# YuePanEdward/MULLS

Hardware: NVIDIA H100
Metric: scan-pair registrations/sec (120k-pt 64-beam) (higher is better)
Workload: dtype f32 geometry / f64 accumulation

## Files before the change

### mulls_b200/csrc/device_types.cuh

```cuda
#pragma once
#include <cstdint>
#include <cuda_runtime.h>

#include "../../include/mulls_b200/abi.h"
#include "search_core.cuh"

namespace mulls {

constexpr int kNumClasses = MULLS_NUM_CLASSES;
constexpr int kNumSegs = 2 * kNumClasses;
constexpr int kIterBlock = 128;
constexpr int kIngestBlock = 256;
constexpr int kTerms = 28;
constexpr int kMaxLevels = 12;
constexpr int kCoordBits = 12;
constexpr int kDedupMinSrc = 500;
constexpr unsigned kClaimFree = 0x7f7f7f7fu;
constexpr int kIterFlags = 256;

enum PairStatus : int { kRunning = 0, kNeedPosterior = 1, kDone = 2 };

struct ChunkDesc {
    uint32_t pair;
    uint32_t seg;
// ... 34 lines not shown
    uint32_t src_index_base[kNumClasses];
    uint32_t src_global_n[kNumClasses];
    int sharded;
};

struct PairState {
    double T_total[16];
    double T_inc[16];
    double x[6];
    double cofactor[36];
    double info[36];
    double sigma2;
    double ibb[6];
    float thre;
    float confidence;
    float origin[3];
    float h0, inv_h0;
    int n_levels;
    int status, code, iter, iters_entered, final_buf;
    int source_feature_points_count;
    int n_src[kNumClasses];
    int n_src_g[kNumClasses];
    int n_src_g_next[kNumClasses];
    int n_tgt[kNumClasses];
    uint32_t n_corr[kNumClasses];
    uint32_t n_corr_last[kNumClasses];
    uint32_t seg_count[kNumSegs];
    uint32_t seg_start[kNumSegs];
    uint32_t hash_entries[kNumClasses];
    uint32_t hash_base[kNumClasses];
    uint32_t hash_mask[kNumClasses];
    int bb_src[6];
    int bb_tgt[6];
    uint64_t alg_bytes;
    int kl_keep[kNumSegs];
    uint32_t kl_rank[kNumSegs];
    uint64_t kl_prefix[kNumSegs];
    uint32_t kl_hist[kNumSegs][256];
};

struct LoopCtl {
    int it;
    int n_it_chunks;
    int n_pairs;
    int trace_on;
    int max_iter;
    unsigned solved;
    unsigned n_live[2];
    unsigned work[4];
};

struct DeviceArrays {
    const float4 *in_aos;
    float4 *stg_pos;
    float4 *stg_nrm;
    uint64_t *keys_a, *keys_b;
    uint32_t *vals_a, *vals_b;
    float4 *tgt_pos, *tgt_nrm;
    float4 *src_pos[2], *src_nrm[2];
    int *src_prevj[2];
    float4 *src_cert[2];
    int *nn_idx;
    float *nn_d2;
    uint8_t *flags;
    int *corr_j;
    float *corr_w;
    unsigned *claim;
    HashEntry *hash;
    uint32_t hash_pool_entries;
    uint32_t *hash_used;
    uint32_t *blk_kept;
    double *partials;
    double *post_partials;
    PairConst *pc;
    PairState *ps;
    ChunkDesc *in_chunks;
    ChunkDesc *it_chunks;
    mulls_icp_trace *trace;
    int *xch_i32;
    double *xch_f64;
    LoopCtl *ctl;
    uint32_t *live_chunks;
    uint32_t live_stride;
    int *running;
    volatile int *h_running;
    volatile int *h_running_iter;
};

}
```

### mulls_b200/csrc/kernels_ingest.cuh

```cuda
#pragma once
#include "device_math.cuh"
#include "device_types.cuh"

namespace mulls {

template <bool kUndistort>
__global__ void __launch_bounds__(kIngestBlock, kUndistort ? 4 : 6) k_ingest_transform(DeviceArrays A) {
    const ChunkDesc cd = A.in_chunks[blockIdx.x];
    const PairConst &pc = A.pc[cd.pair];
    const uint32_t seg = cd.seg;
    const uint32_t local = cd.first + threadIdx.x;
    const bool valid = local < pc.in_n[seg];
    const bool is_src = seg >= kNumClasses;
    const int cls = seg % kNumClasses;
    float x = 0, y = 0, z = 0;
    if (valid) {
        const size_t gi = (size_t)pc.in_off[seg] + local;
        float nx, ny, nz, intensity, curvature = 0.0f;
        const uint32_t fmt = pc.in_fmt[seg];
        if (fmt == 0u) {
            const float4 *in = pc.in_ptr[seg] + 3 * (size_t)local;
            const float4 a = in[0];
            const float4 b = in[1];
            const float4 c = in[2];
            x = a.x, y = a.y, z = a.z;
            nx = b.x, ny = b.y, nz = b.z;
            intensity = c.x, curvature = c.y;
        } else {
            const float4 *in = pc.in_ptr[seg];
            const float4 a = in[local];
            x = a.x, y = a.y, z = a.z, intensity = a.w;
            if (fmt == 1u) {
                const float *nr = reinterpret_cast<const float *>(in + pc.in_n[seg]) + 3 * (size_t)local;
                nx = nr[0], ny = nr[1], nz = nr[2];
            } else {
                const float4 b = in[(size_t)pc.in_n[seg] + local];
                nx = b.x, ny = b.y, nz = b.z, curvature = b.w;
            }
        }
        if (is_src) {
            const double *t = pc.init;
            int n_apply = 1;
            if (kUndistort && pc.undistort) {
                if (cls == MULLS_VERTEX) {
                    n_apply = 2;
                } else {
                    const float curv = curvature;
                    if (!(curv < 0.0f || (double)curv > 1.0)) {
                        const double s = (double)curv;
                        double scale0, scale1;
                        if (pc.ud_linear) {
                            scale0 = 1.0 - s;
                            scale1 = s;
                        } else {
                            scale0 = sin((1.0 - s) * pc.ud_theta) / pc.ud_sin_theta;
                            scale1 = sin(s * pc.ud_theta) / pc.ud_sin_theta;
                        }
                        if (pc.ud_neg) scale1 = -scale1;
                        const double qx = scale1 * pc.ud_q[0], qy = scale1 * pc.ud_q[1], qz = scale1 * pc.ud_q[2],
                                     qw = scale0 + scale1 * pc.ud_q[3];
                        const double vx = x, vy = y, vz = z;
                        double ux = qy * vz - qz * vy, uy = qz * vx - qx * vz, uz = qx * vy - qy * vx;
                        ux += ux, uy += uy, uz += uz;
                        const double rx = vx + qw * ux + (qy * uz - qz * uy);
                        const double ry = vy + qw * uy + (qz * ux - qx * uz);
                        const double rz = vz + qw * uz + (qx * uy - qy * ux);
                        x = (float)(rx + s * pc.ud_t[0]);
                        y = (float)(ry + s * pc.ud_t[1]);
                        z = (float)(rz + s * pc.ud_t[2]);
                    }
                }
            }
            for (int rep = 0; rep < n_apply; ++rep) {
                const double px = x, py = y, pz = z, qx = nx, qy = ny, qz = nz;
                x = (float)(t[0] * px + t[1] * py + t[2] * pz + t[3]);
                y = (float)(t[4] * px + t[5] * py + t[6] * pz + t[7]);
                z = (float)(t[8] * px + t[9] * py + t[10] * pz + t[11]);
                nx = (float)(t[0] * qx + t[1] * qy + t[2] * qz);
                ny = (float)(t[4] * qx + t[5] * qy + t[6] * qz);
                nz = (float)(t[8] * qx + t[9] * qy + t[10] * qz);
            }
        }
        A.stg_pos[gi] = make_float4(x, y, z, intensity);
        A.stg_nrm[gi] = make_float4(nx, ny, nz, __int_as_float((int)local));
    }
    const bool want = is_src ? (cls == MULLS_GROUND || cls == MULLS_PILLAR || cls == MULLS_FACADE) : true;
    if (!want) return;
    float mn[3] = {valid ? x : FLT_MAX, valid ? y : FLT_MAX, valid ? z : FLT_MAX};
    float mx[3] = {valid ? x : -FLT_MAX, valid ? y : -FLT_MAX, valid ? z : -FLT_MAX};
#pragma unroll
    for (int d = 0; d < 3; ++d)
#pragma unroll
        for (int o = 16; o > 0; o >>= 1) {
            mn[d] = fminf(mn[d], __shfl_xor_sync(0xffffffffu, mn[d], o));
            mx[d] = fmaxf(mx[d], __shfl_xor_sync(0xffffffffu, mx[d], o));
        }
    __shared__ float s_mn[kIngestBlock / 32][3], s_mx[kIngestBlock / 32][3];
    if ((threadIdx.x & 31) == 0) {
#pragma unroll
        for (int d = 0; d < 3; ++d) s_mn[threadIdx.x >> 5][d] = mn[d], s_mx[threadIdx.x >> 5][d] = mx[d];
    }
    __syncthreads();
    if (threadIdx.x < 6) {
        const int d = threadIdx.x % 3;
        const bool is_max = threadIdx.x >= 3;
        float v = is_max ? s_mx[0][d] : s_mn[0][d];
        for (int w = 1; w < kIngestBlock / 32; ++w) v = is_max ? fmaxf(v, s_mx[w][d]) : fminf(v, s_mn[w][d]);
        int *bb = is_src ? A.ps[cd.pair].bb_src : A.ps[cd.pair].bb_tgt;
        if (is_max) atomicMax(&bb[3 + d], float_to_ordered(v));
        else atomicMin(&bb[d], float_to_ordered(v));
    }
}

constexpr float kH0Min = 0.125f;
__global__ void k_pair_setup(DeviceArrays A, int n_pairs) {
    const int p = blockIdx.x * blockDim.x + threadIdx.x;
    if (p >= n_pairs) return;
    const PairConst &pc = A.pc[p];
    PairState &ps = A.ps[p];
    double smin[3], smax[3], tmin[3], tmax[3];
    for (int d = 0; d < 3; ++d) {
        smin[d] = (double)ordered_to_float(ps.bb_src[d]);
        smax[d] = (double)ordered_to_float(ps.bb_src[3 + d]);
        tmin[d] = (double)ordered_to_float(ps.bb_tgt[d]);
        tmax[d] = (double)ordered_to_float(ps.bb_tgt[3 + d]);
    }
    const double big = 1.7976931348623157e308;
    double gmin[3], gmax[3];
    if (pc.apply_filter) {
        const float pad = 1.0f;
        for (int d = 0; d < 3; ++d) {
            double lo = (pc.tbound[d] > smin[d]) ? pc.tbound[d] : smin[d];
            double hi = (pc.tbound[3 + d] < smax[d]) ? pc.tbound[3 + d] : smax[d];
            ps.ibb[d] = lo - (double)pad;
            ps.ibb[3 + d] = hi + (double)pad;
            gmin[d] = fmax(tmin[d], ps.ibb[d]);
            gmax[d] = fmin(tmax[d], ps.ibb[3 + d]);
        }
    } else {
        for (int d = 0; d < 3; ++d) {
            ps.ibb[d] = -big;
            ps.ibb[3 + d] = big;
            gmin[d] = tmin[d];
            gmax[d] = tmax[d];
        }
    }
    double ext = 0.0;
    for (int d = 0; d < 3; ++d) {
        if (!(gmax[d] >= gmin[d])) {
            gmin[d] = 0.0;
            gmax[d] = 0.0;
        }
        ext = fmax(ext, gmax[d] - gmin[d]);
    }
    const int ncell = 1 << kCoordBits;
    float h0 = kH0Min;
    while ((ext + 8.0 * h0) * 1.001 > (double)h0 * (ncell - 4)) h0 *= 2.0f;
    ps.h0 = h0;
    ps.inv_h0 = 1.0f / h0;
    for (int d = 0; d < 3; ++d) ps.origin[d] = (float)gmin[d] - 2.0f * h0;
    const float rmax = 2.5f * pc.thre_unit * 1.0001f;
    int L = 2;
    while (L < kMaxLevels && 0.999f * 0.5f * h0 * (float)(1 << (L - 1)) < rmax) ++L;
    if (pc.normal_shooting) L = kMaxLevels;
    ps.n_levels = L;

    for (int i = 0; i < 16; ++i) {
        ps.T_total[i] = pc.init[i];
        ps.T_inc[i] = (i % 5 == 0) ? 1.0 : 0.0;
    }
    for (int i = 0; i < 36; ++i) ps.cofactor[i] = ps.info[i] = (i % 7 == 0) ? 1.0 : 0.0;
    for (int i = 0; i < 6; ++i) ps.x[i] = 0.0;
    ps.sigma2 = 1.0;
    ps.thre = pc.thre_unit;
    ps.confidence = 1.0f;
    ps.status = kRunning;
    ps.code = 0;
    ps.iter = 0;
    ps.iters_entered = 0;
    ps.final_buf = 0;
    ps.alg_bytes = 0;
    if (pc.max_iter <= 0) {
        ps.status = kDone;
        const int left = atomicSub(A.running, 1) - 1;
        *A.h_running = left;
        __threadfence_system();
    }
}

__global__ void __launch_bounds__(kIngestBlock) k_make_keys(DeviceArrays A) {
    const ChunkDesc cd = A.in_chunks[blockIdx.x];
    const PairConst &pc = A.pc[cd.pair];
    PairState &ps = A.ps[cd.pair];
    const uint32_t seg = cd.seg;
    const uint32_t local = cd.first + threadIdx.x;
    const bool valid = local < pc.in_n[seg];
    bool inside = false;
    if (valid) {
        const size_t gi = (size_t)pc.in_off[seg] + local;
        const float4 p = A.stg_pos[gi];
        const double *b = ps.ibb;
        inside = (double)p.x > b[0] && (double)p.x < b[3] && (double)p.y > b[1] && (double)p.y < b[4] &&
                 (double)p.z > b[2] && (double)p.z < b[5];
        uint64_t key = ~0ull;
        if (inside) {
            const int hi = (1 << kCoordBits) - 1;
            int cx = (int)floorf((p.x - ps.origin[0]) * ps.inv_h0);
            int cy = (int)floorf((p.y - ps.origin[1]) * ps.inv_h0);
            int cz = (int)floorf((p.z - ps.origin[2]) * ps.inv_h0);
            cx = min(max(cx, 0), hi);
            cy = min(max(cy, 0), hi);
            cz = min(max(cz, 0), hi);
            key = ((uint64_t)(cd.pair * kNumSegs + seg) << 36) | morton36((uint32_t)cx, (uint32_t)cy, (uint32_t)cz);
        }
        A.keys_a[gi] = key;
        A.vals_a[gi] = (uint32_t)gi;
    }
    const unsigned ballot = __ballot_sync(0xffffffffu, inside);
    if ((threadIdx.x & 31) == 0 && ballot) atomicAdd(&ps.seg_count[seg], (unsigned)__popc(ballot));
}

__device__ __forceinline__ uint64_t sample_key(uint32_t seed, uint32_t cloud_id, uint32_t index) {
    uint64_t z = (((uint64_t)seed << 40) ^ ((uint64_t)cloud_id << 32) ^ (uint64_t)index) + 0x9e3779b97f4a7c15ull;
    z = (z ^ (z >> 30)) * 0xbf58476d1ce4e5b9ull;
    z = (z ^ (z >> 27)) * 0x94d049bb133111ebull;
    return z ^ (z >> 31);
}

__global__ void k_keepless_plan(DeviceArrays A, int n_pairs) {
    const int p = blockIdx.x * blockDim.x + threadIdx.x;
    if (p >= n_pairs) return;
    const PairConst &pc = A.pc[p];
    PairState &ps = A.ps[p];
    for (int s = 0; s < kNumSegs; ++s) {
        ps.kl_keep[s] = -1;
        ps.kl_prefix[s] = 0;
        ps.kl_rank[s] = 0;
        for (int b = 0; b < 256; ++b) ps.kl_hist[s][b] = 0;
    }
    if (!pc.keep_less) return;
    const int S = kNumClasses;
    auto plan = [&](int seg, int keep) {
        if ((int)ps.seg_count[seg] > keep) {
            ps.kl_keep[seg] = keep;
            ps.kl_rank[seg] = (uint32_t)keep;
        }
        return ((int)ps.seg_count[seg] > keep) ? keep : (int)ps.seg_count[seg];
    };
    const int tg = plan(MULLS_GROUND, (int)(ps.seg_count[MULLS_GROUND] / 2));
    const int tf = plan(MULLS_FACADE, (int)(ps.seg_count[MULLS_FACADE] / 2));
    plan(S + MULLS_GROUND, tg / 4);
    plan(S + MULLS_FACADE, tf / 2);
    plan(S + MULLS_PILLAR, (int)ps.seg_count[MULLS_PILLAR]);
// ... 65 lines not shown
}

__global__ void k_seg_offsets(DeviceArrays A, int n_pairs) {
    __shared__ uint32_t carry;
    __shared__ uint32_t warp_sums[32];
    if (threadIdx.x == 0) carry = 0;
    __syncthreads();
    const int total = n_pairs * kNumSegs;
    for (int base = 0; base < total; base += blockDim.x) {
        const int i = base + threadIdx.x;
        uint32_t v = 0;
        if (i < total) v = A.ps[i / kNumSegs].seg_count[i % kNumSegs];
        uint32_t incl = v;
        for (int o = 1; o < 32; o <<= 1) {
            uint32_t t = __shfl_up_sync(0xffffffffu, incl, o);
            if ((threadIdx.x & 31) >= o) incl += t;
        }
        if ((threadIdx.x & 31) == 31) warp_sums[threadIdx.x >> 5] = incl;
        __syncthreads();
        if (threadIdx.x < 32) {
            uint32_t w = (threadIdx.x < (blockDim.x >> 5)) ? warp_sums[threadIdx.x] : 0;
            uint32_t wi = w;
            for (int o = 1; o < 32; o <<= 1) {
                uint32_t t = __shfl_up_sync(0xffffffffu, wi, o);
                if (threadIdx.x >= o) wi += t;
            }
            warp_sums[threadIdx.x] = wi - w;
        }
        __syncthreads();
        const uint32_t excl = carry + warp_sums[threadIdx.x >> 5] + incl - v;
        if (i < total) A.ps[i / kNumSegs].seg_start[i % kNumSegs] = excl;
        __syncthreads();
        if (threadIdx.x == blockDim.x - 1) carry = excl + v;
        __syncthreads();
    }
    for (int p = threadIdx.x; p < n_pairs; p += blockDim.x) {
        PairState &ps = A.ps[p];
        const PairConst &pc = A.pc[p];
        for (int c = 0; c < kNumClasses; ++c) {
            ps.n_tgt[c] = (int)ps.seg_count[c];
            ps.n_src[c] = (int)ps.seg_count[kNumClasses + c];
            ps.n_src_g[c] = ps.n_src[c];
            ps.n_corr[c] = 0;
            ps.n_corr_last[c] = 0;
        }
        int cnt = 0;
        if (pc.used[MULLS_PILLAR]) cnt += ps.n_src[MULLS_PILLAR];
        if (pc.used[MULLS_FACADE]) cnt += ps.n_src[MULLS_FACADE];
        if (pc.used[MULLS_BEAM]) cnt += ps.n_src[MULLS_BEAM];
        ps.source_feature_points_count = cnt;
    }
}

__global__ void __launch_bounds__(256) k_gather(DeviceArrays A, const uint64_t *keys, const uint32_t *vals, uint32_t n_total) {
    const uint32_t i = blockIdx.x * blockDim.x + threadIdx.x;
    if (i >= n_total) return;
    const uint64_t key = keys[i];
    if (key == ~0ull) return;
    const uint32_t sg = (uint32_t)(key >> 36);
    const uint32_t pair = sg / kNumSegs, seg = sg % kNumSegs;
    const PairConst &pc = A.pc[pair];
    const uint32_t local = i - A.ps[pair].seg_start[seg];
    const uint32_t v = vals[i];
    const float4 pos = A.stg_pos[v];
    const float4 nrm = A.stg_nrm[v];
    if (seg < kNumClasses) {
        const uint32_t d = pc.tgt_base[seg] + local;
        A.tgt_pos[d] = pos;
        A.tgt_nrm[d] = nrm;
    } else {
        const uint32_t d = pc.src_base[seg - kNumClasses] + local;
        float4 n2 = nrm;
        if (pc.sharded) n2.w = __int_as_float(__float_as_int(nrm.w) + (int)pc.src_index_base[seg - kNumClasses]);
        A.src_pos[0][d] = pos;
        A.src_nrm[0][d] = n2;
        A.src_prevj[0][d] = -1;
        A.src_cert[0][d] = make_float4(0.f, 0.f, 0.f, 0.f);
    }
}

__device__ __forceinline__ void hash_insert(HashEntry *table, uint32_t mask, uint32_t klo, uint32_t khi, uint32_t start) {
    uint32_t slot = cell_hash(klo, khi) & mask;
    const unsigned long long packed = (unsigned long long)klo | ((unsigned long long)khi << 32);
    while (true) {
        unsigned long long *kp = reinterpret_cast<unsigned long long *>(&table[slot]);
        unsigned long long old = atomicCAS(kp, 0ull, packed);
        if (old == 0ull) {
            table[slot].start = start;
            return;
        }
        slot = (slot + 1) & mask;
    }
}
__device__ __forceinline__ HashEntry *hash_find(HashEntry *table, uint32_t mask, uint32_t klo, uint32_t khi) {
    uint32_t slot = cell_hash(klo, khi) & mask;
    while (true) {
        const uint32_t lo = *reinterpret_cast<volatile uint32_t *>(&table[slot].key_lo);
        const uint32_t hi = *reinterpret_cast<volatile uint32_t *>(&table[slot].key_hi);
        if (lo == klo && (hi & kKeyHiMask) == khi) return &table[slot];
        if (lo == 0u && hi == 0u) return nullptr;
        slot = (slot + 1) & mask;
    }
}

__global__ void __launch_bounds__(256) k_hash_build(DeviceArrays A, const uint64_t *keys, uint32_t n_total, int mode) {
    const uint32_t i = blockIdx.x * blockDim.x + threadIdx.x;
    const bool in_range = i <= n_total;
    const uint64_t kcur = (in_range && i < n_total) ? keys[i] : ~0ull;
    const uint64_t kprev = (in_range && i > 0) ? keys[i - 1] : ~0ull;
    const bool cur_t = kcur != ~0ull && ((uint32_t)(kcur >> 36) % kNumSegs) < kNumClasses;
    const bool prev_t = kprev != ~0ull && ((uint32_t)(kprev >> 36) % kNumSegs) < kNumClasses;
    const bool same_seg = cur_t && prev_t && (kcur >> 36) == (kprev >> 36);
    const uint64_t mmask = (1ull << 36) - 1;
    int top = kMaxLevels - 1;
    bool boundary = true;
    if (same_seg) {
        const uint64_t diff = (kcur ^ kprev) & mmask;
        if (diff == 0) boundary = false;
        else top = (63 - __clzll((long long)diff)) / 3;
    }
    if (mode == 0) {
        uint32_t sg = cur_t ? (uint32_t)(kcur >> 36) : 0xffffffffu;
        int cnt = 0;
        if (cur_t && boundary) {
            const int L = A.ps[sg / kNumSegs].n_levels;
            cnt = min(top, L - 1) + 1;
        }
        const unsigned grp = __match_any_sync(0xffffffffu, sg);
        if (grp == 0xffffffffu) {
            const int tot = __reduce_add_sync(0xffffffffu, cnt);
            if ((threadIdx.x & 31) == 0 && tot > 0 && cur_t)
                atomicAdd(&A.ps[sg / kNumSegs].hash_entries[sg % kNumSegs], (unsigned)tot);
        } else if (cnt > 0) {
            atomicAdd(&A.ps[sg / kNumSegs].hash_entries[sg % kNumSegs], (unsigned)cnt);
        }
        return;
    }
    if (!boundary || A.hash_used[1]) return;
    if (mode == 1) {
        if (!cur_t) return;
        const uint32_t sg = (uint32_t)(kcur >> 36);
        const uint32_t pair = sg / kNumSegs, cls = sg % kNumSegs;
        const PairState &ps = A.ps[pair];
        const int L = ps.n_levels;
        const uint32_t local = i - ps.seg_start[cls];
        HashEntry *table = A.hash + ps.hash_base[cls];
        const uint64_t m = kcur & mmask;
        const uint32_t x0 = compact12(m), y0 = compact12(m >> 1), z0 = compact12(m >> 2);
        for (int l = 0; l <= top && l < L; ++l)
            hash_insert(table, ps.hash_mask[cls], cell_key_lo(x0 >> l, y0 >> l, z0 >> l), cell_key_hi(z0 >> l, l), local);
    } else {
        if (!prev_t) return;
        const uint32_t sg = (uint32_t)(kprev >> 36);
        const uint32_t pair = sg / kNumSegs, cls = sg % kNumSegs;
        const PairState &ps = A.ps[pair];
        const int L = ps.n_levels;
        const uint32_t local_end = i - ps.seg_start[cls];
        HashEntry *table = A.hash + ps.hash_base[cls];
        const uint64_t m = kprev & mmask;
        const uint32_t x0 = compact12(m), y0 = compact12(m >> 1), z0 = compact12(m >> 2);
        for (int l = 0; l <= top && l < L; ++l) {
            const uint32_t x = x0 >> l, y = y0 >> l, z = z0 >> l;
            HashEntry *e = hash_find(table, ps.hash_mask[cls], cell_key_lo(x, y, z), cell_key_hi(z, l));
            if (e) e->count = local_end - e->start;
            if (l + 1 < L) {
                HashEntry *par = hash_find(table, ps.hash_mask[cls], cell_key_lo(x >> 1, y >> 1, z >> 1), cell_key_hi(z >> 1, l + 1));
                if (par) atomicOr(&par->key_hi, 1u << (16 + ((x & 1u) | ((y & 1u) << 1) | ((z & 1u) << 2))));
            }
        }
    }
}

constexpr uint64_t kHashSlack = 4;
__global__ void k_hash_layout(DeviceArrays A, int n_pairs) {
    if (threadIdx.x != 0 || blockIdx.x != 0) return;
    for (int attempt = 0; attempt < 3; ++attempt) {
        uint64_t used = 0;
        bool overflow = false;
        for (int p = 0; p < n_pairs && !overflow; ++p) {
            PairState &ps = A.ps[p];
            for (int c = 0; c < kNumClasses; ++c) {
                const uint64_t want = (attempt == 0) ? kHashSlack * ps.hash_entries[c] : (attempt == 1) ? 2ull * ps.hash_entries[c] : (5ull * ps.hash_entries[c]) / 4 + 1;
                uint32_t cap = 16;
                while (cap < want) cap <<= 1;
                if (used + cap > A.hash_pool_entries) {
                    overflow = true;
                    break;
                }
                ps.hash_base[c] = (uint32_t)used;
                ps.hash_mask[c] = cap - 1;
                used += cap;
            }
        }
        A.hash_used[0] = overflow ? 0u : (uint32_t)used;
        A.hash_used[1] = overflow ? 1u : 0u;
        if (!overflow) return;
    }
    for (int p = 0; p < n_pairs; ++p)
        for (int c = 0; c < kNumClasses; ++c) {
            A.ps[p].hash_base[c] = 0;
            A.ps[p].hash_mask[c] = 0;
        }
}

__global__ void __launch_bounds__(256) k_hash_clear(DeviceArrays A) {
    const uint32_t used = A.hash_used[0];
    const uint4 z = make_uint4(0, 0, 0, 0);
    for (uint32_t i = blockIdx.x * blockDim.x + threadIdx.x; i < used; i += gridDim.x * blockDim.x)
        reinterpret_cast<uint4 *>(A.hash)[i] = z;
}

}
```

### mulls_b200/csrc/mulls_b200.cu

```cuda
#include <algorithm>
#include <atomic>
#include <memory>
#include <cmath>
#include <cstdio>
#include <chrono>
#include <cstring>
#include <string>
#include <vector>

#include <cub/device/device_radix_sort.cuh>
#include <cub/device/device_scan.cuh>

#include <dlfcn.h>
#include <mutex>

#include "device_types.cuh"
#include "host_pack.h"
#include "scan_io.h"
#include "kernels_ingest.cuh"
#include "kernels_iterate.cuh"
#include "kernels_pca.cuh"
#include "kernels_map.cuh"
#include "kernels_classify.cuh"
#include "kernels_ground.cuh"
// ... 189 lines not shown
    if (ctx->graph) cudaGraphDestroy(ctx->graph);
    if (ctx->h_stage) cudaFreeHost(ctx->h_stage);
    for (cudaEvent_t e : ctx->ev_done) cudaEventDestroy(e);
    for (cudaEvent_t e : ctx->ev_search) cudaEventDestroy(e);
    if (ctx->ev_begin) cudaEventDestroy(ctx->ev_begin);
    if (ctx->ev_ingest) cudaEventDestroy(ctx->ev_ingest);
    if (ctx->ev_iter) cudaEventDestroy(ctx->ev_iter);
    if (ctx->ev_end) cudaEventDestroy(ctx->ev_end);
    if (ctx->ev_h2d0) cudaEventDestroy(ctx->ev_h2d0);
    if (ctx->stream) cudaStreamDestroy(ctx->stream);
    delete ctx;
}

mulls_ctx *mulls_create(int device, size_t max_pairs, size_t max_src_pts, size_t max_tgt_pts) {
    int ndev = 0;
    cudaError_t e = cudaGetDeviceCount(&ndev);
    if (e != cudaSuccess || ndev == 0) {
        g_create_error = std::string("mulls_create: no CUDA device (") + cudaGetErrorString(e) +
                         "); mulls_b200 has no CPU fallback";
        return nullptr;
    }
    if (device < 0 || device >= ndev || max_pairs == 0) {
        g_create_error = "mulls_create: bad device index or max_pairs";
        return nullptr;
    }
    mulls_ctx *ctx = new mulls_ctx();
    ctx->device = device;
    ctx->max_pairs = max_pairs;
    ctx->max_src = max_src_pts;
    ctx->max_tgt = max_tgt_pts;
    auto fail = [&](const char *what, cudaError_t err) -> mulls_ctx * {
        g_create_error = std::string("mulls_create: ") + what + ": " + cudaGetErrorString(err);
        mulls_destroy(ctx);
        return nullptr;
    };
    if ((e = cudaSetDevice(device)) != cudaSuccess) return fail("cudaSetDevice", e);
    if ((e = cudaStreamCreateWithFlags(&ctx->stream, cudaStreamNonBlocking)) != cudaSuccess) return fail("stream", e);
    const size_t cs = ctx->cap_src = max_pairs * max_src_pts;
    const size_t ct = ctx->cap_tgt = max_pairs * max_tgt_pts;
    const size_t cin = ctx->cap_in = cs + ct;
    if (cin >= (1ull << 31)) {
        g_create_error = "mulls_create: more than 2^31 points per context";
        mulls_destroy(ctx);
        return nullptr;
    }
    ctx->cap_it_chunks = ceil_div(cs, kIterBlock) + max_pairs * (kNumClasses + 1);
    ctx->cap_in_chunks = ceil_div(cin, kIngestBlock) + max_pairs * kNumSegs;
    DeviceArrays &A = ctx->A;
    float4 *in = nullptr;
#define ALLOC(ptr, n)                                                   \
    if ((e = dev_alloc(ctx, &(ptr), (n))) != cudaSuccess) return fail(#ptr, e)
    ALLOC(in, 3 * cin);
    A.in_aos = in;
    ALLOC(A.stg_pos, cin);
    ALLOC(A.stg_nrm, cin);
    ALLOC(A.keys_a, cin);
    ALLOC(A.keys_b, cin);
    ALLOC(A.vals_a, cin);
    ALLOC(A.vals_b, cin);
    ALLOC(A.tgt_pos, ct + kScanOverrun);
    ALLOC(A.tgt_nrm, ct);
    for (int b = 0; b < 2; ++b) {
        ALLOC(A.src_pos[b], cs);
        ALLOC(A.src_nrm[b], cs);
        ALLOC(A.src_prevj[b], cs);
        ALLOC(A.src_cert[b], cs);
    }
    ALLOC(A.nn_idx, cs);
    ALLOC(A.nn_d2, cs);
    ALLOC(A.flags, cs);
    ALLOC(A.corr_j, cs);
    ALLOC(A.corr_w, cs);
    ALLOC(A.claim, ct);
    {
        size_t pool = 12 * ct + 64 * max_pairs * kNumClasses;
        if (pool >= (1ull << 32)) pool = (1ull << 32) - 1;
        A.hash_pool_entries = (uint32_t)pool;
        ALLOC(A.hash, pool);
    }
    ALLOC(A.hash_used, 2);
    ALLOC(A.ctl, 1);
    ALLOC(A.blk_kept, ctx->cap_it_chunks);
    ALLOC(A.partials, ctx->cap_it_chunks * kTerms);
    ALLOC(A.post_partials, ctx->cap_it_chunks * 2);
    ALLOC(A.pc, max_pairs);
    ALLOC(A.ps, max_pairs);
    ALLOC(A.in_chunks, ctx->cap_in_chunks);
    ALLOC(A.it_chunks, ctx->cap_it_chunks);
    ALLOC(A.live_chunks, 2 * ctx->cap_it_chunks);
    A.live_stride = (uint32_t)ctx->cap_it_chunks;
    {
        int sms = 0;
        if (cudaDeviceGetAttribute(&sms, cudaDevAttrMultiProcessorCount, device) != cudaSuccess || sms <= 0) sms = 132;
        ctx->num_sms = sms;
    }
    ALLOC(ctx->d_results, max_pairs + ceil_div(max_pairs * sizeof(uint64_t), sizeof(mulls_icp_result)) + 1);
    ALLOC(ctx->d_trace, max_pairs);
    ALLOC(A.running, 1);
    ALLOC(A.xch_i32, 32);
    ALLOC(A.xch_f64, kNumClasses * kTerms + 8);
#undef ALLOC
    if ((e = cudaHostAlloc((void **)&ctx->h_running, (1 + kIterFlags) * sizeof(int), cudaHostAllocMapped)) != cudaSuccess)
        return fail("mapped flag", e);
    {
        int *dptr = nullptr;
        if ((e = cudaHostGetDevicePointer((void **)&dptr, ctx->h_running, 0)) != cudaSuccess) return fail("mapped flag", e);
        A.h_running = dptr;
        A.h_running_iter = dptr + 1;
// ... 312 lines not shown
        CK(ce);
    } else {
    if (cudaEventRecord(ctx->ev_h2d0, ctx->stream) == cudaSuccess) ctx->h2d_timed = true;
    for (size_t p = 0; p < n_pairs; ++p) {
        PairConst &pc = ctx->h_pc[p];
        for (int s = 0; s < kNumSegs; ++s) {
            const mulls_cloud_view &v = (s < kNumClasses) ? tgt[p * kNumClasses + s] : src[p * kNumClasses + (s - kNumClasses)];
            pc.in_ptr[s] = ctx->A.in_aos + 3 * (size_t)pc.in_off[s];
            pc.in_fmt[s] = kFmtRows48;
            if (v.n == 0) continue;
            if (tgt_on_device && s < kNumClasses) {
                pc.in_ptr[s] = (const float4 *)v.aos48;
                continue;
            }
            CK(cudaMemcpyAsync((void *)(ctx->A.in_aos + 3 * (size_t)pc.in_off[s]), v.aos48, v.n * 48, cudaMemcpyHostToDevice,
                               ctx->stream));
        }
    }
    }
    if (!tables_sent) {
        CK(cudaMemcpyAsync(ctx->A.pc, ctx->h_pc.data(), n_pairs * sizeof(PairConst), cudaMemcpyHostToDevice, ctx->stream));
        if (!ctx->h_in_chunks.empty())
            CK(cudaMemcpyAsync(ctx->A.in_chunks, ctx->h_in_chunks.data(), ctx->h_in_chunks.size() * sizeof(ChunkDesc),
                               cudaMemcpyHostToDevice, ctx->stream));
        if (!ctx->h_it_chunks.empty())
            CK(cudaMemcpyAsync(ctx->A.it_chunks, ctx->h_it_chunks.data(), ctx->h_it_chunks.size() * sizeof(ChunkDesc),
                               cudaMemcpyHostToDevice, ctx->stream));
    }
    if (resident) CK(cudaStreamSynchronize(ctx->stream));
    ctx->n_pairs = n_pairs;
    ctx->n_in = in_off;
    ctx->n_src_total = s_off;
    ctx->n_tgt_total = t_off;
    ctx->max_iter_max = max_iter_max;
    ctx->any_keep_less = any_keep_less;
    ctx->any_normal_shooting = any_shoot;
    ctx->any_undistort = any_undistort;
    ctx->uploaded = true;
    ctx->up_ms_host = (float)(wall_ms() - t_up0);
    return MULLS_OK;
}

static int launch_ingest(mulls_ctx *ctx, DeviceArrays &A, bool trace, uint64_t &launches, mulls_allreduce_fn hook = nullptr,
                         void *user = nullptr) {
    cudaStream_t st = ctx->stream;
    const int np = (int)ctx->n_pairs;
    const uint32_t n_in = (uint32_t)ctx->n_in;
    if (trace) CK(cudaMemsetAsync(ctx->d_trace, 0, np * sizeof(mulls_icp_trace), st));
    CK(cudaMemsetAsync(A.claim, 0x7f, std::max<size_t>(ctx->n_tgt_total, 1) * sizeof(unsigned), st));
    k_state_init<<<(unsigned)ceil_div(np, 128), 128, 0, st>>>(A, np);
    ++launches;
    const unsigned n_inc = (unsigned)ctx->h_in_chunks.size();
    if (n_inc) {
        if (ctx->any_undistort) k_ingest_transform<true><<<n_inc, kIngestBlock, 0, st>>>(A);
        else k_ingest_transform<false><<<n_inc, kIngestBlock, 0, st>>>(A);
        ++launches;
    }
    if (hook) {
        k_shard_pack_setup<<<1, 1, 0, st>>>(A, 0);
        if (hook(user, A.xch_i32, 6, 1, 1, (void *)st) != 0) {
            ctx->err = "all-reduce callback failed";
            return MULLS_E_COMM;
        }
        k_shard_pack_setup<<<1, 1, 0, st>>>(A, 1);
        launches += 2;
    }
    k_pair_setup<<<(unsigned)ceil_div(np, 128), 128, 0, st>>>(A, np);
    ++launches;
    if (n_inc) {
        k_make_keys<<<n_inc, kIngestBlock, 0, st>>>(A);
        ++launches;
        if (ctx->any_keep_less) {
            const unsigned pb = (unsigned)ceil_div(np, 64);
            k_keepless_plan<<<pb, 64, 0, st>>>(A, np);
            for (int pass = 0; pass < 8; ++pass) {
                k_keepless_hist<<<n_inc, kIngestBlock, 0, st>>>(A, pass);
                k_keepless_step<<<pb, 64, 0, st>>>(A, np, pass);
            }
            k_keepless_mark<<<n_inc, kIngestBlock, 0, st>>>(A);
            launches += 18;
        }
        int seg_bits = 1;
        while ((1ull << seg_bits) <= (uint64_t)np * kNumSegs) ++seg_bits;
        size_t bytes = ctx->cub_temp_bytes;
        CK(cub::DeviceRadixSort::SortPairs(ctx->cub_temp, bytes, A.keys_a, A.keys_b, A.vals_a, A.vals_b, (int)n_in, 0,
                                           36 + seg_bits, st));
    }
    k_seg_offsets<<<1, 256, 0, st>>>(A, np);
    ++launches;
    if (hook) {
        k_shard_pack_setup<<<1, 1, 0, st>>>(A, 2);
        if (hook(user, A.xch_i32, kNumClasses, 1, 0, (void *)st) != 0) {
            ctx->err = "all-reduce callback failed";
            return MULLS_E_COMM;
        }
        k_shard_pack_setup<<<1, 1, 0, st>>>(A, 3);
        launches += 2;
    }
    if (n_in) {
        k_gather<<<(unsigned)ceil_div(n_in, 256), 256, 0, st>>>(A, A.keys_b, A.vals_b, n_in);
        const unsigned hb = (unsigned)ceil_div((size_t)n_in + 1, 256);
        k_hash_build<<<hb, 256, 0, st>>>(A, A.keys_b, n_in, 0);
        k_hash_layout<<<1, 32, 0, st>>>(A, np);
        k_hash_clear<<<1184, 256, 0, st>>>(A);
        k_hash_build<<<hb, 256, 0, st>>>(A, A.keys_b, n_in, 1);
        k_hash_build<<<hb, 256, 0, st>>>(A, A.keys_b, n_in, 2);
        launches += 6;
    } else {
        k_hash_layout<<<1, 32, 0, st>>>(A, np);
        ++launches;
    }
    return MULLS_OK;
}

static unsigned chunk_bucket(const mulls_ctx *ctx) {
    unsigned b = 1;
    while (b < (unsigned)ctx->h_it_chunks.size()) b <<= 1;
    return b;
}
static unsigned resident_grid(const mulls_ctx *ctx, int blocks_per_sm) {
    return std::min((unsigned)(ctx->num_sms * blocks_per_sm), chunk_bucket(ctx));
}
static void launch_search(mulls_ctx *ctx, cudaStream_t st, const DeviceArrays &A, int buf, int it) {
    const unsigned grid = resident_grid(ctx, kSearchBlocksPerSm);
    const int mode = it < 0 ? -1 : (it >= kKeepFromIter ? 2 : (it == kKeepFromIter - 1 ? 1 : 0));
    if (mode < 0 || mode == 0) k_search<0><<<grid, kIterBlock, 0, st>>>(A, buf, it);
    if (mode < 0 || mode == 1) k_search<1><<<grid, kIterBlock, 0, st>>>(A, buf, it);
    if (mode < 0 || mode == 2) k_search<2><<<grid, kIterBlock, 0, st>>>(A, buf, it);
}
constexpr int kShootBlocksPerSm = 8, kResolveBlocksPerSm = 16, kAccumulateBlocksPerSm = 8;
constexpr int kPollPause = 64;

static int build_iteration_graph(mulls_ctx *ctx) {
    const int key[2] = {(int)chunk_bucket(ctx), ctx->any_normal_shooting ? 1 : 0};
    if (ctx->graph_exec && std::memcmp(key, ctx->graph_key, sizeof(key)) == 0) return MULLS_OK;
    if (ctx->graph_exec) cudaGraphExecDestroy(ctx->graph_exec), ctx->graph_exec = nullptr;
    if (ctx->graph) cudaGraphDestroy(ctx->graph), ctx->graph = nullptr;
    cudaStream_t st = ctx->stream;
    DeviceArrays A = ctx->A;
    const unsigned cap_chunks = (unsigned)std::max<size_t>(ctx->cap_it_chunks, 1), cap_pairs = (unsigned)std::max<size_t>(ctx->max_pairs, 1);
    CK(cudaGraphCreate(&ctx->graph, 0));
    cudaGraphConditionalHandle handle;
    CK(cudaGraphConditionalHandleCreate(&handle, ctx->graph, 1, cudaGraphCondAssignDefault));
    cudaGraphNodeParams wp = {cudaGraphNodeTypeConditional};
    wp.conditional.handle = handle;
    wp.conditional.type = cudaGraphCondTypeWhile;
    wp.conditional.size = 1;
    cudaGraphNode_t while_node;
    CK(cudaGraphAddNode(&while_node, ctx->graph, nullptr, 0, &wp));
    cudaGraph_t body = wp.conditional.phGraph_out[0];
    CK(cudaStreamBeginCaptureToGraph(st, body, nullptr, nullptr, 0, cudaStreamCaptureModeThreadLocal));
    launch_search(ctx, st, A, -1, -1);
    if (ctx->any_normal_shooting)
        k_search_shoot<<<resident_grid(ctx, kShootBlocksPerSm), kIterBlock, 0, st>>>(A, -1);
    k_resolve<<<resident_grid(ctx, kResolveBlocksPerSm), kIterBlock, 0, st>>>(A, -1);
    k_accumulate<<<resident_grid(ctx, kAccumulateBlocksPerSm), kIterBlock, 0, st>>>(A, -1);
    k_solve<<<cap_pairs, kSolveThreads, 0, st>>>(A, -1, (unsigned long long)handle);
    CK(cudaStreamEndCapture(st, nullptr));
    CK(cudaStreamBeginCaptureToGraph(st, ctx->graph, &while_node, nullptr, 1, cudaStreamCaptureModeThreadLocal));
    k_posterior<<<std::min(cap_chunks, chunk_bucket(ctx)), kIterBlock, 0, st>>>(A);
// ... 1301 lines not shown
```

Baseline: 5954.

## Drop staging buffers, recompute transforms on demand, and build hash in one pass

After: 6250 (median of 6 runs). +5.0%, better.

```diff
diff --git a/mulls_b200/csrc/device_types.cuh b/mulls_b200/csrc/device_types.cuh
--- a/mulls_b200/csrc/device_types.cuh
+++ b/mulls_b200/csrc/device_types.cuh
@@ -110,8 +110,6 @@
 
 struct DeviceArrays {
     const float4 *in_aos;
-    float4 *stg_pos;
-    float4 *stg_nrm;
     uint64_t *keys_a, *keys_b;
     uint32_t *vals_a, *vals_b;
     float4 *tgt_pos, *tgt_nrm;
diff --git a/mulls_b200/csrc/kernels_ingest.cuh b/mulls_b200/csrc/kernels_ingest.cuh
--- a/mulls_b200/csrc/kernels_ingest.cuh
+++ b/mulls_b200/csrc/kernels_ingest.cuh
@@ -4,90 +4,107 @@
 
 namespace mulls {
 
-template <bool kUndistort>
-__global__ void __launch_bounds__(kIngestBlock, kUndistort ? 4 : 6) k_ingest_transform(DeviceArrays A) {
-    const ChunkDesc cd = A.in_chunks[blockIdx.x];
-    const PairConst &pc = A.pc[cd.pair];
-    const uint32_t seg = cd.seg;
-    const uint32_t local = cd.first + threadIdx.x;
-    const bool valid = local < pc.in_n[seg];
+template <bool kUndistort, bool kNormals>
+__device__ __forceinline__ void load_input_point(const PairConst &pc, uint32_t seg, uint32_t local, float4 &pos, float4 &nrm) {
     const bool is_src = seg >= kNumClasses;
     const int cls = seg % kNumClasses;
-    float x = 0, y = 0, z = 0;
-    if (valid) {
-        const size_t gi = (size_t)pc.in_off[seg] + local;
-        float nx, ny, nz, intensity, curvature = 0.0f;
-        const uint32_t fmt = pc.in_fmt[seg];
-        if (fmt == 0u) {
-            const float4 *in = pc.in_ptr[seg] + 3 * (size_t)local;
-            const float4 a = in[0];
+    const bool undistort = kUndistort && is_src && pc.undistort && cls != MULLS_VERTEX;
+    float x, y, z, intensity = 0.0f, curvature = 0.0f;
+    float nx = 0.0f, ny = 0.0f, nz = 0.0f;
+    const uint32_t fmt = pc.in_fmt[seg];
+    if (fmt == 0u) {
+        const float4 *in = pc.in_ptr[seg] + 3 * (size_t)local;
+        const float4 a = in[0];
+        x = a.x, y = a.y, z = a.z;
+        if (kNormals) {
             const float4 b = in[1];
             const float4 c = in[2];
-            x = a.x, y = a.y, z = a.z;
             nx = b.x, ny = b.y, nz = b.z;
             intensity = c.x, curvature = c.y;
-        } else {
-            const float4 *in = pc.in_ptr[seg];
-            const float4 a = in[local];
-            x = a.x, y = a.y, z = a.z, intensity = a.w;
-            if (fmt == 1u) {
+        } else if (undistort) {
+            curvature = reinterpret_cast<const float *>(in + 2)[1];
+        }
+    } else {
+        const float4 *in = pc.in_ptr[seg];
+        const float4 a = in[local];
+        x = a.x, y = a.y, z = a.z, intensity = a.w;
+        if (fmt == 1u) {
+            if (kNormals) {
                 const float *nr = reinterpret_cast<const float *>(in + pc.in_n[seg]) + 3 * (size_t)local;
                 nx = nr[0], ny = nr[1], nz = nr[2];
+            }
+        } else if (kNormals) {
+            const float4 b = in[(size_t)pc.in_n[seg] + local];
+            nx = b.x, ny = b.y, nz = b.z, curvature = b.w;
+        } else if (undistort) {
+            curvature = in[(size_t)pc.in_n[seg] + local].w;
+        }
+    }
+    if (is_src) {
+        const double *t = pc.init;
+        int n_apply = 1;
+        if (kUndistort && pc.undistort) {
+            if (cls == MULLS_VERTEX) {
+                n_apply = 2;
             } else {
-                const float4 b = in[(size_t)pc.in_n[seg] + local];
-                nx = b.x, ny = b.y, nz = b.z, curvature = b.w;
-            }
-        }
-        if (is_src) {
-            const double *t = pc.init;
-            int n_apply = 1;
-            if (kUndistort && pc.undistort) {
-                if (cls == MULLS_VERTEX) {
-                    n_apply = 2;
-                } else {
-                    const float curv = curvature;
-                    if (!(curv < 0.0f || (double)curv > 1.0)) {
-                        const double s = (double)curv;
-                        double scale0, scale1;
-                        if (pc.ud_linear) {
-                            scale0 = 1.0 - s;
-                            scale1 = s;
-                        } else {
-                            scale0 = sin((1.0 - s) * pc.ud_theta) / pc.ud_sin_theta;
-                            scale1 = sin(s * pc.ud_theta) / pc.ud_sin_theta;
-                        }
-                        if (pc.ud_neg) scale1 = -scale1;
-                        const double qx = scale1 * pc.ud_q[0], qy = scale1 * pc.ud_q[1], qz = scale1 * pc.ud_q[2],
-                                     qw = scale0 + scale1 * pc.ud_q[3];
-                        const double vx = x, vy = y, vz = z;
-                        double ux = qy * vz - qz * vy, uy = qz * vx - qx * vz, uz = qx * vy - qy * vx;
-                        ux += ux, uy += uy, uz += uz;
-                        const double rx = vx + qw * ux + (qy * uz - qz * uy);
-                        const double ry = vy + qw * uy + (qz * ux - qx * uz);
-                        const double rz = vz + qw * uz + (qx * uy - qy * ux);
-                        x = (float)(rx + s * pc.ud_t[0]);
-                        y = (float)(ry + s * pc.ud_t[1]);
-                        z = (float)(rz + s * pc.ud_t[2]);
+                const float curv = curvature;
+                if (!(curv < 0.0f || (double)curv > 1.0)) {
+                    const double s = (double)curv;
+                    double scale0, scale1;
+                    if (pc.ud_linear) {
+                        scale0 = 1.0 - s;
+                        scale1 = s;
+                    } else {
+                        scale0 = sin((1.0 - s) * pc.ud_theta) / pc.ud_sin_theta;
+                        scale1 = sin(s * pc.ud_theta) / pc.ud_sin_theta;
                     }
+                    if (pc.ud_neg) scale1 = -scale1;
+                    const double qx = scale1 * pc.ud_q[0], qy = scale1 * pc.ud_q[1], qz = scale1 * pc.ud_q[2],
+                                 qw = scale0 + scale1 * pc.ud_q[3];
+                    const double vx = x, vy = y, vz = z;
+                    double ux = qy * vz - qz * vy, uy = qz * vx - qx * vz, uz = qx * vy - qy * vx;
+                    ux += ux, uy += uy, uz += uz;
+                    const double rx = vx + qw * ux + (qy * uz - qz * uy);
+                    const double ry = vy + qw * uy + (qz * ux - qx * uz);
+                    const double rz = vz + qw * uz + (qx * uy - qy * ux);
+                    x = (float)(rx + s * pc.ud_t[0]);
+                    y = (float)(ry + s * pc.ud_t[1]);
+                    z = (float)(rz + s * pc.ud_t[2]);
                 }
             }
-            for (int rep = 0; rep < n_apply; ++rep) {
-                const double px = x, py = y, pz = z, qx = nx, qy = ny, qz = nz;
-                x = (float)(t[0] * px + t[1] * py + t[2] * pz + t[3]);
-                y = (float)(t[4] * px + t[5] * py + t[6] * pz + t[7]);
-                z = (float)(t[8] * px + t[9] * py + t[10] * pz + t[11]);
+        }
+        for (int rep = 0; rep < n_apply; ++rep) {
+            const double px = x, py = y, pz = z;
+            x = (float)(t[0] * px + t[1] * py + t[2] * pz + t[3]);
+            y = (float)(t[4] * px + t[5] * py + t[6] * pz + t[7]);
+            z = (float)(t[8] * px + t[9] * py + t[10] * pz + t[11]);
+            if (kNormals) {
+                const double qx = nx, qy = ny, qz = nz;
                 nx = (float)(t[0] * qx + t[1] * qy + t[2] * qz);
                 ny = (float)(t[4] * qx + t[5] * qy + t[6] * qz);
                 nz = (float)(t[8] * qx + t[9] * qy + t[10] * qz);
             }
         }
-        A.stg_pos[gi] = make_float4(x, y, z, intensity);
-        A.stg_nrm[gi] = make_float4(nx, ny, nz, __int_as_float((int)local));
-    }
+    }
+    pos = make_float4(x, y, z, intensity);
+    if (kNormals) nrm = make_float4(nx, ny, nz, __int_as_float((int)local));
+}
+
+template <bool kUndistort>
+__global__ void __launch_bounds__(kIngestBlock) k_ingest_bbox(DeviceArrays A) {
+    const ChunkDesc cd = A.in_chunks[blockIdx.x];
+    const PairConst &pc = A.pc[cd.pair];
+    const uint32_t seg = cd.seg;
+    const bool is_src = seg >= kNumClasses;
+    const int cls = seg % kNumClasses;
     const bool want = is_src ? (cls == MULLS_GROUND || cls == MULLS_PILLAR || cls == MULLS_FACADE) : true;
     if (!want) return;
-    float mn[3] = {valid ? x : FLT_MAX, valid ? y : FLT_MAX, valid ? z : FLT_MAX};
-    float mx[3] = {valid ? x : -FLT_MAX, valid ? y : -FLT_MAX, valid ? z : -FLT_MAX};
+    const uint32_t local = cd.first + threadIdx.x;
+    const bool valid = local < pc.in_n[seg];
+    float4 p = make_float4(0.f, 0.f, 0.f, 0.f), unused;
+    if (valid) load_input_point<kUndistort, false>(pc, seg, local, p, unused);
+    float mn[3] = {valid ? p.x : FLT_MAX, valid ? p.y : FLT_MAX, valid ? p.z : FLT_MAX};
+    float mx[3] = {valid ? p.x : -FLT_MAX, valid ? p.y : -FLT_MAX, valid ? p.z : -FLT_MAX};
 #pragma unroll
     for (int d = 0; d < 3; ++d)
 #pragma unroll
@@ -188,6 +205,7 @@
     }
 }
 
+template <bool kUndistort>
 __global__ void __launch_bounds__(kIngestBlock) k_make_keys(DeviceArrays A) {
     const ChunkDesc cd = A.in_chunks[blockIdx.x];
     const PairConst &pc = A.pc[cd.pair];
@@ -198,7 +216,8 @@
     bool inside = false;
     if (valid) {
         const size_t gi = (size_t)pc.in_off[seg] + local;
-        const float4 p = A.stg_pos[gi];
+        float4 p, unused;
+        load_input_point<kUndistort, false>(pc, seg, local, p, unused);
         const double *b = ps.ibb;
         inside = (double)p.x > b[0] && (double)p.x < b[3] && (double)p.y > b[1] && (double)p.y < b[4] &&
                  (double)p.z > b[2] && (double)p.z < b[5];
@@ -370,122 +389,114 @@
     }
 }
 
+__device__ __forceinline__ int cell_top(const uint64_t *keys, uint32_t i, uint64_t kcur) {
+    if (kcur == ~0ull || ((uint32_t)(kcur >> 36) % kNumSegs) >= kNumClasses) return -1;
+    if (i == 0) return kMaxLevels - 1;
+    const uint64_t kprev = keys[i - 1];
+    if ((kprev >> 36) != (kcur >> 36)) return kMaxLevels - 1;
+    const uint64_t diff = (kcur ^ kprev) & ((1ull << 36) - 1);
+    if (diff == 0) return -1;
+    return (63 - __clzll((long long)diff)) / 3;
+}
+
+template <bool kUndistort>
 __global__ void __launch_bounds__(256) k_gather(DeviceArrays A, const uint64_t *keys, const uint32_t *vals, uint32_t n_total) {
     const uint32_t i = blockIdx.x * blockDim.x + threadIdx.x;
-    if (i >= n_total) return;
-    const uint64_t key = keys[i];
-    if (key == ~0ull) return;
+    const uint64_t key = i < n_total ? keys[i] : ~0ull;
     const uint32_t sg = (uint32_t)(key >> 36);
     const uint32_t pair = sg / kNumSegs, seg = sg % kNumSegs;
+    const int top = cell_top(keys, i, key);
+    const int cnt = top < 0 ? 0 : min(top, A.ps[pair].n_levels - 1) + 1;
+    const bool is_tgt = key != ~0ull && seg < kNumClasses;
+    const unsigned grp = __match_any_sync(0xffffffffu, is_tgt ? sg : 0xffffffffu);
+    if (grp == 0xffffffffu) {
+        const int tot = __reduce_add_sync(0xffffffffu, cnt);
+        if ((threadIdx.x & 31) == 0 && tot > 0) atomicAdd(&A.ps[pair].hash_entries[seg], (unsigned)tot);
+    } else if (cnt > 0) {
+        atomicAdd(&A.ps[pair].hash_entries[seg], (unsigned)cnt);
+    }
+    if (key == ~0ull) return;
     const PairConst &pc = A.pc[pair];
+    float4 pos, nrm;
+    load_input_point<kUndistort, true>(pc, seg, vals[i] - pc.in_off[seg], pos, nrm);
     const uint32_t local = i - A.ps[pair].seg_start[seg];
-    const uint32_t v = vals[i];
-    const float4 pos = A.stg_pos[v];
-    const float4 nrm = A.stg_nrm[v];
     if (seg < kNumClasses) {
         const uint32_t d = pc.tgt_base[seg] + local;
         A.tgt_pos[d] = pos;
         A.tgt_nrm[d] = nrm;
     } else {
         const uint32_t d = pc.src_base[seg - kNumClasses] + local;
-        float4 n2 = nrm;
-        if (pc.sharded) n2.w = __int_as_float(__float_as_int(nrm.w) + (int)pc.src_index_base[seg - kNumClasses]);
+        if (pc.sharded) nrm.w = __int_as_float(__float_as_int(nrm.w) + (int)pc.src_index_base[seg - kNumClasses]);
         A.src_pos[0][d] = pos;
-        A.src_nrm[0][d] = n2;
+        A.src_nrm[0][d] = nrm;
         A.src_prevj[0][d] = -1;
         A.src_cert[0][d] = make_float4(0.f, 0.f, 0.f, 0.f);
     }
 }
 
-__device__ __forceinline__ void hash_insert(HashEntry *table, uint32_t mask, uint32_t klo, uint32_t khi, uint32_t start) {
-    uint32_t slot = cell_hash(klo, khi) & mask;
-    const unsigned long long packed = (unsigned long long)klo | ((unsigned long long)khi << 32);
+__device__ __forceinline__ void hash_insert(HashEntry *table, uint32_t hmask, uint32_t klo, uint32_t khi, uint32_t children,
+                                            uint32_t start, uint32_t count) {
+    uint32_t slot = cell_hash(klo, khi) & hmask;
+    const unsigned long long packed = (unsigned long long)klo | ((unsigned long long)(khi | (children << 16)) << 32);
     while (true) {
         unsigned long long *kp = reinterpret_cast<unsigned long long *>(&table[slot]);
-        unsigned long long old = atomicCAS(kp, 0ull, packed);
-        if (old == 0ull) {
-            table[slot].start = start;
+        if (atomicCAS(kp, 0ull, packed) == 0ull) {
+            *reinterpret_cast<uint2 *>(&table[slot].start) = make_uint2(start, count);
             return;
         }
-        slot = (slot + 1) & mask;
-    }
-}
-__device__ __forceinline__ HashEntry *hash_find(HashEntry *table, uint32_t mask, uint32_t klo, uint32_t khi) {
-    uint32_t slot = cell_hash(klo, khi) & mask;
-    while (true) {
-        const uint32_t lo = *reinterpret_cast<volatile uint32_t *>(&table[slot].key_lo);
-        const uint32_t hi = *reinterpret_cast<volatile uint32_t *>(&table[slot].key_hi);
-        if (lo == klo && (hi & kKeyHiMask) == khi) return &table[slot];
-        if (lo == 0u && hi == 0u) return nullptr;
-        slot = (slot + 1) & mask;
-    }
-}
-
-__global__ void __launch_bounds__(256) k_hash_build(DeviceArrays A, const uint64_t *keys, uint32_t n_total, int mode) {
+        slot = (slot + 1) & hmask;
+    }
+}
+
+__device__ __forceinline__ uint32_t cell_end(const uint64_t *keys, uint32_t b, uint32_t hi, uint64_t p, int shift) {
+    uint32_t in = b, out = hi, step = 1;
+    while (in + step < hi) {
+        if ((keys[in + step] >> shift) != p) {
+            out = in + step;
+            break;
+        }
+        in += step;
+        step <<= 1;
+    }
+    while (out - in > 1) {
+        const uint32_t mid = in + (out - in) / 2;
+        if ((keys[mid] >> shift) == p) in = mid;
+        else out = mid;
+    }
+    return out;
+}
+
+__global__ void __launch_bounds__(256) k_hash_build(DeviceArrays A, const uint64_t *keys, uint32_t n_total) {
     const uint32_t i = blockIdx.x * blockDim.x + threadIdx.x;
-    const bool in_range = i <= n_total;
-    const uint64_t kcur = (in_range && i < n_total) ? keys[i] : ~0ull;
-    const uint64_t kprev = (in_range && i > 0) ? keys[i - 1] : ~0ull;
-    const bool cur_t = kcur != ~0ull && ((uint32_t)(kcur >> 36) % kNumSegs) < kNumClasses;
-    const bool prev_t = kprev != ~0ull && ((uint32_t)(kprev >> 36) % kNumSegs) < kNumClasses;
-    const bool same_seg = cur_t && prev_t && (kcur >> 36) == (kprev >> 36);
-    const uint64_t mmask = (1ull << 36) - 1;
-    int top = kMaxLevels - 1;
-    bool boundary = true;
-    if (same_seg) {
-        const uint64_t diff = (kcur ^ kprev) & mmask;
-        if (diff == 0) boundary = false;
-        else top = (63 - __clzll((long long)diff)) / 3;
-    }
-    if (mode == 0) {
-        uint32_t sg = cur_t ? (uint32_t)(kcur >> 36) : 0xffffffffu;
-        int cnt = 0;
-        if (cur_t && boundary) {
-            const int L = A.ps[sg / kNumSegs].n_levels;
-            cnt = min(top, L - 1) + 1;
-        }
-        const unsigned grp = __match_any_sync(0xffffffffu, sg);
-        if (grp == 0xffffffffu) {
-            const int tot = __reduce_add_sync(0xffffffffu, cnt);
-            if ((threadIdx.x & 31) == 0 && tot > 0 && cur_t)
-                atomicAdd(&A.ps[sg / kNumSegs].hash_entries[sg % kNumSegs], (unsigned)tot);
-        } else if (cnt > 0) {
-            atomicAdd(&A.ps[sg / kNumSegs].hash_entries[sg % kNumSegs], (unsigned)cnt);
-        }
-        return;
-    }
-    if (!boundary || A.hash_used[1]) return;
-    if (mode == 1) {
-        if (!cur_t) return;
-        const uint32_t sg = (uint32_t)(kcur >> 36);
-        const uint32_t pair = sg / kNumSegs, cls = sg % kNumSegs;
-        const PairState &ps = A.ps[pair];
-        const int L = ps.n_levels;
-        const uint32_t local = i - ps.seg_start[cls];
-        HashEntry *table = A.hash + ps.hash_base[cls];
-        const uint64_t m = kcur & mmask;
-        const uint32_t x0 = compact12(m), y0 = compact12(m >> 1), z0 = compact12(m >> 2);
-        for (int l = 0; l <= top && l < L; ++l)
-            hash_insert(table, ps.hash_mask[cls], cell_key_lo(x0 >> l, y0 >> l, z0 >> l), cell_key_hi(z0 >> l, l), local);
-    } else {
-        if (!prev_t) return;
-        const uint32_t sg = (uint32_t)(kprev >> 36);
-        const uint32_t pair = sg / kNumSegs, cls = sg % kNumSegs;
-        const PairState &ps = A.ps[pair];
-        const int L = ps.n_levels;
-        const uint32_t local_end = i - ps.seg_start[cls];
-        HashEntry *table = A.hash + ps.hash_base[cls];
-        const uint64_t m = kprev & mmask;
-        const uint32_t x0 = compact12(m), y0 = compact12(m >> 1), z0 = compact12(m >> 2);
-        for (int l = 0; l <= top && l < L; ++l) {
-            const uint32_t x = x0 >> l, y = y0 >> l, z = z0 >> l;
-            HashEntry *e = hash_find(table, ps.hash_mask[cls], cell_key_lo(x, y, z), cell_key_hi(z, l));
-            if (e) e->count = local_end - e->start;
-            if (l + 1 < L) {
-                HashEntry *par = hash_find(table, ps.hash_mask[cls], cell_key_lo(x >> 1, y >> 1, z >> 1), cell_key_hi(z >> 1, l + 1));
-                if (par) atomicOr(&par->key_hi, 1u << (16 + ((x & 1u) | ((y & 1u) << 1) | ((z & 1u) << 2))));
+    if (i >= n_total || A.hash_used[1]) return;
+    const uint64_t kcur = keys[i];
+    const int top = cell_top(keys, i, kcur);
+    if (top < 0) return;
+    const uint32_t sg = (uint32_t)(kcur >> 36);
+    const uint32_t pair = sg / kNumSegs, cls = sg % kNumSegs;
+    const PairState &ps = A.ps[pair];
+    const int L = ps.n_levels;
+    const uint32_t seg_begin = ps.seg_start[cls], seg_end = seg_begin + ps.seg_count[cls];
+    HashEntry *table = A.hash + ps.hash_base[cls];
+    const uint32_t hmask = ps.hash_mask[cls];
+    const uint64_t m = kcur & ((1ull << 36) - 1);
+    const uint32_t x0 = compact12(m), y0 = compact12(m >> 1), z0 = compact12(m >> 2);
+    uint32_t end = cell_end(keys, i, seg_end, kcur, 0);
+    for (int l = 0; l <= top && l < L; ++l) {
+        uint32_t children = 0;
+        if (l > 0) {
+            const int shift = 3 * l;
+            const uint64_t p = kcur >> shift;
+            children = 1u << ((kcur >> (shift - 3)) & 7u);
+            while (end < seg_end) {
+                const uint64_t k = keys[end];
+                if ((k >> shift) != p) break;
+                children |= 1u << ((k >> (shift - 3)) & 7u);
+                end = cell_end(keys, end, seg_end, k >> (shift - 3), shift - 3);
             }
         }
+        const uint32_t x = x0 >> l, y = y0 >> l, z = z0 >> l;
+        hash_insert(table, hmask, cell_key_lo(x, y, z), cell_key_hi(z, l), children, i - seg_begin, end - i);
     }
 }
 
diff --git a/mulls_b200/csrc/mulls_b200.cu b/mulls_b200/csrc/mulls_b200.cu
--- a/mulls_b200/csrc/mulls_b200.cu
+++ b/mulls_b200/csrc/mulls_b200.cu
@@ -265,8 +265,6 @@
     if ((e = dev_alloc(ctx, &(ptr), (n))) != cudaSuccess) return fail(#ptr, e)
     ALLOC(in, 3 * cin);
     A.in_aos = in;
-    ALLOC(A.stg_pos, cin);
-    ALLOC(A.stg_nrm, cin);
     ALLOC(A.keys_a, cin);
     ALLOC(A.keys_b, cin);
     ALLOC(A.vals_a, cin);
@@ -685,8 +683,8 @@
     ++launches;
     const unsigned n_inc = (unsigned)ctx->h_in_chunks.size();
     if (n_inc) {
-        if (ctx->any_undistort) k_ingest_transform<true><<<n_inc, kIngestBlock, 0, st>>>(A);
-        else k_ingest_transform<false><<<n_inc, kIngestBlock, 0, st>>>(A);
+        if (ctx->any_undistort) k_ingest_bbox<true><<<n_inc, kIngestBlock, 0, st>>>(A);
+        else k_ingest_bbox<false><<<n_inc, kIngestBlock, 0, st>>>(A);
         ++launches;
     }
     if (hook) {
@@ -701,7 +699,8 @@
     k_pair_setup<<<(unsigned)ceil_div(np, 128), 128, 0, st>>>(A, np);
     ++launches;
     if (n_inc) {
-        k_make_keys<<<n_inc, kIngestBlock, 0, st>>>(A);
+        if (ctx->any_undistort) k_make_keys<true><<<n_inc, kIngestBlock, 0, st>>>(A);
+        else k_make_keys<false><<<n_inc, kIngestBlock, 0, st>>>(A);
         ++launches;
         if (ctx->any_keep_less) {
             const unsigned pb = (unsigned)ceil_div(np, 64);
@@ -731,14 +730,13 @@
         launches += 2;
     }
     if (n_in) {
-        k_gather<<<(unsigned)ceil_div(n_in, 256), 256, 0, st>>>(A, A.keys_b, A.vals_b, n_in);
-        const unsigned hb = (unsigned)ceil_div((size_t)n_in + 1, 256);
-        k_hash_build<<<hb, 256, 0, st>>>(A, A.keys_b, n_in, 0);
+        const unsigned nb = (unsigned)ceil_div(n_in, 256);
+        if (ctx->any_undistort) k_gather<true><<<nb, 256, 0, st>>>(A, A.keys_b, A.vals_b, n_in);
+        else k_gather<false><<<nb, 256, 0, st>>>(A, A.keys_b, A.vals_b, n_in);
         k_hash_layout<<<1, 32, 0, st>>>(A, np);
         k_hash_clear<<<1184, 256, 0, st>>>(A);
-        k_hash_build<<<hb, 256, 0, st>>>(A, A.keys_b, n_in, 1);
-        k_hash_build<<<hb, 256, 0, st>>>(A, A.keys_b, n_in, 2);
-        launches += 6;
+        k_hash_build<<<nb, 256, 0, st>>>(A, A.keys_b, n_in);
+        launches += 4;
     } else {
         k_hash_layout<<<1, 32, 0, st>>>(A, np);
         ++launches;
```
